# tk1363704/CAREL-VAE

Hardware: AMD Instinct MI355X
Metric: clause-pairs/sec (training step) (higher is better)
Workload: dtype bf16

## Files before the change

carel_vae_amd/csrc/carel_hip_internal.h:

```cpp
#pragma once
#include <hip/hip_runtime.h>
#include <stdarg.h>
#include <stdio.h>
#include "../../include/carel_hip.h"
#include "carel_common.h"

#ifdef CAREL_EXPERIMENTS
#define CAREL_TUNABLE(type, name, value) static type name = value
#else
#define CAREL_TUNABLE(type, name, value) static constexpr type name = value
#endif

namespace carel {

int set_error(int code, const char* fmt, ...);
int check_launch(const char* what);
int slab_reduce_multi(const void* slabs, void* out, int64_t n, const void* slabs2, void* out2, int64_t n2, int splits, const void* partials,
                      int nparts, void* dgamma, void* dbeta, void* dbias, hipStream_t stream);
#ifdef CAREL_EXPERIMENTS
int gemm_rowln_wanted(long rows);
int gemm_rowln_wanted_k(int K);
#else
inline int gemm_rowln_wanted(long) { return 0; }
inline int gemm_rowln_wanted_k(int) { return 0; }
#endif
void encoder_ln_resid_enable(int on);
void encoder_ln_slab_fusion_enable(int on);
void encoder_wgrad_group_enable(int on);
void adam_grid_cap(long cap);
void tail_overlap_enable(int on);
int gemm_pp_init_device(int device);
int gather_rows(const void* in_f32, const void* in_bf16, const void* idx, int n, void* out_f32, void* out_bf16, hipStream_t stream);
int scatter_rows(const void* in_f32, const void* in_bf16, const void* idx, int n, void* out_f32, void* out_bf16, hipStream_t stream);

int layernorm_bwd_rows(const void* dy, const void* h, const void* stats, const void* gamma, int64_t rows, uint32_t drop_seed, uint32_t drop_site,
                       uint32_t drop_idx_offset, float drop_p, const void* drop_row_map, void* dh_f32, void* dy_bf16, void* partials,
                       hipStream_t stream);
int layernorm_bwd_reduce(const void* partials, int64_t rows, void* dgamma, void* dbeta, void* dbias, hipStream_t stream);
int layernorm_bwd_blocks_max(int64_t rows);
int layernorm_bwd_rows_slabs(const void* slabs, int splits, const void* resid, const void* h, const void* stats, const void* gamma, int64_t rows,
                             uint32_t drop_seed, uint32_t drop_site, uint32_t drop_idx_offset, float drop_p, const void* drop_row_map, void* dh_f32,
                             void* dy_bf16, void* partials, hipStream_t stream);
int layernorm_fwd_slabs(const void* slabs, int splits, const void* bias, const void* resid, const void* resid_stats, const void* resid_gamma,
                        const void* resid_beta, uint32_t drop_seed, uint32_t drop_site, uint32_t drop_idx_offset, float drop_p, const void* drop_row_map,
                        void* h_out, const void* gamma, const void* beta, float eps, int64_t rows, void* x_f32, void* x_bf16, void* stats,
                        hipStream_t stream);

constexpr int GEMM_EX_FIXED_ROWS = 0x100;
constexpr int GEMM_EX_DEFER_EPILOGUE = 0x200;
int gemm_bf16_ex(const carel_gemm_args* a, int split_tile_factor, void* stream);
int gemm_bf16_split_plan(const carel_gemm_args* a, int split_tile_factor);
int gemm_wgrad_splits_max(int M, int N, long T);
int embed_ln_bwd_ex(const carel_embed_args* a, const void* dx0, void* dword, void* dpos, void* dtype_, void* dgamma, void* dbeta,
                    void* partials, void* row_scratch, hipStream_t stream, const void* sort_ws = nullptr);
int embed_sort_supported(const carel_embed_args* a);
size_t embed_sort_bytes();
int embed_ln_fwd_keys(const carel_embed_args* a, void* sort_ws, hipStream_t stream);
int embed_sort_rows(const carel_embed_args* a, void* sort_ws, hipStream_t stream);

struct WgradGroupProb { const void* dY; const void* X; void* dW; void* db; int M, N; };
struct WgradGroupLn { const void* partials; int nparts; void* dgamma; void* dbeta; void* dbias; };
size_t gemm_pp_wgrad_group_ws_bytes(const WgradGroupProb* pb, int n, long T);
int gemm_pp_wgrad_group_ok(const WgradGroupProb* pb, int n, long T);
int gemm_pp_wgrad_group(const WgradGroupProb* pb, int n, long T, void* ws, size_t ws_bytes, const WgradGroupLn* ln, int n_ln, hipStream_t stream);

inline Dropout make_dropout(uint32_t seed, uint32_t site, float p, uint32_t idx_offset) {
  Dropout d;
  d.key = mix32(seed + site * 0x9E3779B9u);
  d.idx_offset = idx_offset;
  if (p <= 0.f) { d.thresh = 0u; d.scale = 1.f; }
  else if (p >= 1.f) { d.thresh = 0xFFFFFFFFu; d.scale = 0.f; }
  else {
    d.thresh = (uint32_t)((double)p * 4294967296.0);
    d.scale = (float)(1.0 / (1.0 - (double)p));
    if (d.thresh == 0u) d.scale = 1.f;
  }
  return d;
}

struct AttnParams;
int attn_long_fwd(const AttnParams& q, hipStream_t stream);
int attn_long_bwd(const AttnParams& q, void* workspace, int64_t workspace_bytes, hipStream_t stream);

}
```

carel_vae_amd/csrc/encoder.hip:

```cpp
#include <cstdlib>
#include <mutex>
#include <vector>
#include "carel_hip_internal.h"

using namespace carel;

namespace {

constexpr int EH = 768, EI = 3072, ENH = 12;

size_t al(size_t x) { return (x + 255) & ~(size_t)255; }

struct LayerAct {
  char* xin_bf16; char* qkv; char* lse; char* ctx; char* h1; char* st1; char* x1_bf16; char* u; char* g; char* h2; char* st2;
};
struct ActLayout {
  size_t per_layer, total;
  size_t o_xin, o_qkv, o_lse, o_ctx, o_h1, o_st1, o_x1, o_u, o_g, o_h2, o_st2;
  size_t o_embst, o_xa, o_xb, o_cctx, o_cxres, o_layers;
};

ActLayout act_layout(long B, long S, int L, int inference) {
  const size_t T = (size_t)B * S;
  ActLayout a; size_t o = 0;
// ... 303 lines not shown
    char* next_bf16 = nullptr;
    if (i + 1 < a->n_layers) next_bf16 = layer_act(l, base, i + 1, a->inference).xin_bf16 + (size_t)r0 * EH * 2;
    if (fuse_ln && gemm_rowln_wanted_k(EI)) {
      if ((rc = linear_ln(la.g, w.ffn2_w, EI, w.ffn2_b, xb, 3 + 3 * i, w.ln2_g, w.ln2_b, a->inference ? nullptr : la.h2, xa, next_bf16, la.st2))) return rc;
    } else if ((rc = linear_then_ln(la.g, w.ffn2_w, EI, w.ffn2_b, lnres2 ? (const void*)la.h1 : (const void*)xb, lnres2 ? &lr2 : nullptr, 3 + 3 * i, w.ln2_g,
                                    w.ln2_b, la.h2, need_xa ? xa : nullptr, next_bf16, la.st2))) return rc;
  }
  return CAREL_OK;
}

struct EmbedKeyRecord { const void* scratch; const void* act; const void* ids; const void* tok_row; long rows; bool side; };
static std::mutex g_key_mu;
static std::vector<EmbedKeyRecord> g_key_records;

static long embed_rows_of(const carel_embed_args& e) { return (e.tok_row && e.n_rows > 0) ? (long)e.n_rows : (long)e.batch * e.seq_len; }

static void embed_keys_written(const carel_encoder_args* a, const carel_embed_args* e, bool keys, bool side) {
  std::lock_guard<std::mutex> lk(g_key_mu);
  std::vector<EmbedKeyRecord>& r = g_key_records;
  for (size_t i = 0; i < r.size();)
    if (r[i].act == a->act || (keys && r[i].scratch == a->scratch)) { r[i] = r.back(); r.pop_back(); } else ++i;
  if (keys) r.push_back(EmbedKeyRecord{a->scratch, a->act, a->input_ids, a->tok_row, embed_rows_of(*e), side});
}

static int embed_keys_match(const carel_encoder_args* a, const carel_embed_args* e, bool* side) {
  std::lock_guard<std::mutex> lk(g_key_mu);
  for (const EmbedKeyRecord& k : g_key_records)
    if (k.scratch == a->scratch) {
      *side = k.side;
      return k.act == a->act && k.ids == a->input_ids && k.tok_row == a->tok_row && k.rows == embed_rows_of(*e);
    }
  return 0;
}

extern "C" int carel_encoder_forward(const carel_encoder_args* a, void* stream) {
  int rc = enc_check(a, "carel_encoder_forward");
  if (rc) return rc;
  if (!a->word_emb || !a->pos_emb || !a->type_emb || !a->emb_ln_g || !a->emb_ln_b) return set_error(CAREL_ERR_ARG, "carel_encoder_forward: null embedding tensor");
  const long B = a->batch, S = a->seq_len;
  const ActLayout l = act_layout(B, S, a->n_layers, a->inference);
  const ScratchLayout sl = scratch_layout(B, S);
  char* ws = a->scratch ? (char*)a->scratch + sl.o_ws : nullptr;
  const size_t ws_bytes = a->scratch ? sl.ws_bytes : 0;
  LayerAct la = layer_act(l, (char*)a->act, 0, a->inference);
  carel_embed_args e = embed_args_of(a, l, la);
  if (!a->inference && a->scratch && embed_sort_supported(&e)) {
    void* sort_ws = (char*)a->scratch + sl.o_sort;
    if ((rc = embed_ln_fwd_keys(&e, sort_ws, (hipStream_t)stream))) return rc;
    SideStream* ss = ((a->overlap_wgrad & 1) && !(a->overlap_wgrad & 2)) ? side_stream() : nullptr;
    if (ss) {
      if (hipEventRecord(ss->ev[8], (hipStream_t)stream) != hipSuccess || hipStreamWaitEvent(ss->stream, ss->ev[8], 0) != hipSuccess)
        return set_error(CAREL_ERR_HIP, "carel_encoder_forward: event fork failed");
      if ((rc = embed_sort_rows(&e, sort_ws, ss->stream))) return rc;
    } else if ((rc = embed_sort_rows(&e, sort_ws, (hipStream_t)stream))) return rc;
    embed_keys_written(a, &e, true, ss != nullptr);
  } else {
    embed_keys_written(a, &e, false, false);
    if ((rc = carel_embed_ln_fwd(&e, stream))) return rc;
  }
  const long hb = B / 2;
  const int lsplit = a->n_cls > 0 ? a->n_layers - 1 : a->n_layers;
  SideStream* sd = nullptr;
  if ((a->overlap_wgrad & 2) && !a->tok_row && (B & 1) == 0 && (hb * S) % 128 == 0 && lsplit >= 1 && a->scratch) sd = side_stream();
  if (!sd) return forward_layers(a, 0, a->n_layers, 0, B, stream, ws, ws_bytes);
  if (hipEventRecord(sd->ev[0], (hipStream_t)stream) != hipSuccess || hipStreamWaitEvent(sd->peer, sd->ev[0], 0) != hipSuccess)
    return set_error(CAREL_ERR_HIP, "carel_encoder_forward: event fork failed");
  char* ws2 = (char*)a->scratch + sl.o_slabs;
  rc = forward_layers(a, 0, lsplit, hb, hb, (void*)sd->peer, ws2, sl.ws_bytes, 2);
  if (!rc) rc = forward_layers(a, 0, lsplit, 0, hb, stream, ws, ws_bytes, 2);
  if (rc) return rc;
  if (hipEventRecord(sd->ev[1], sd->peer) != hipSuccess || hipStreamWaitEvent((hipStream_t)stream, sd->ev[1], 0) != hipSuccess)
    return set_error(CAREL_ERR_HIP, "carel_encoder_forward: event join failed");
  if (lsplit < a->n_layers) return forward_layers(a, lsplit, a->n_layers, 0, B, stream, ws, ws_bytes);
  return CAREL_OK;
}

extern "C" int carel_encoder_backward_layer(const carel_encoder_args* a, int32_t layer, void* stream) {
  int rc = enc_check(a, "carel_encoder_backward_layer");
  if (rc) return rc;
  if (a->inference) return set_error(CAREL_ERR_ARG, "carel_encoder_backward_layer: forward ran in inference mode (no saved activations)");
  if (layer < 0 || layer >= a->n_layers || !a->layer_grads || !a->scratch || !a->dx)
    return set_error(CAREL_ERR_ARG, "carel_encoder_backward_layer: bad layer index or null buffer");
  const long B = a->batch, S = a->seq_len, T = n_rows_of(a);
  const ActLayout l = act_layout(B, S, a->n_layers, 0);
  const LayerAct la = layer_act(l, (char*)a->act, layer, 0);
  const ScratchLayout sl = scratch_layout(B, S);
  const int par = layer & 1;
  const Scratch s = scratch_of(sl, (char*)a->scratch, par);
  const carel_layer_params& w = a->layers[layer];
  const carel_layer_grads& g = a->layer_grads[layer];
  const uint32_t hoff = a->drop_row_offset * (uint32_t)(S * EH), aoff = a->drop_row_offset * (uint32_t)(ENH * S * S);
  const size_t ws_bytes = sl.ws_bytes;
  SideStream* sd = nullptr;
  if (a->overlap_wgrad & 1) {
    sd = side_stream();
    if (!sd) return set_error(CAREL_ERR_HIP, "carel_encoder_backward_layer: could not create the side stream / events");
  }
  void* wstream = sd ? (void*)sd->stream : stream;
  int nfork = 0;
  auto fork = [&]() -> int {
    if (!sd) return CAREL_OK;
    hipEvent_t ev = sd->ev[nfork++];
    if (hipEventRecord(ev, (hipStream_t)stream) != hipSuccess || hipStreamWaitEvent(sd->stream, ev, 0) != hipSuccess)
      return set_error(CAREL_ERR_HIP, "carel_encoder_backward_layer: event fork failed");
    return CAREL_OK;
  };
// ... 18 lines not shown
  ga.ln[0] = carel_ln_partial_set{s.part, R, g.ln2_g, g.ln2_b, g.ffn2_b};
  ga.ln[1] = carel_ln_partial_set{s.part3, R, g.ln1_g, g.ln1_b, g.out_b};
  ga.n_ln = 2;
  bool grouped = false;
  if (wgrad_group_enabled() && !cls_only) {
    const int64_t need = carel_gemm_wgrad_group_ws_bytes(&ga);
    grouped = need >= 0 && need <= (int64_t)sl.slab_bytes;
  }
  GemmCall gqkv = gemm_fill(s.dqkv, w.qkv_w, 3 * EH, EH, (int)T, EH, 3 * EH, CAREL_GEMM_NN, CAREL_EPI_ADD_F32, 1, nullptr, nullptr, a->dx, nullptr, s.dy,
                            nullptr, 0, 0, 0, 0.f, nullptr, nullptr, s.ws, ws_bytes, 1);
  const int qkv_slabs = ln_slab_fusion_enabled() ? gemm_bf16_split_plan(&gqkv.g, gqkv.flags) : 1;
  const bool dx_in_slabs = qkv_slabs > 1 && layer + 1 < a->n_layers && !(a->n_cls > 0 && layer + 2 == a->n_layers);
  if ((rc = wait_group(0))) return rc;
  if (dx_in_slabs) {
    if ((rc = layernorm_bwd_rows_slabs(s.ws, qkv_slabs, s.dy, la.h2, la.st2, w.ln2_g, R, a->drop_seed, 3 + 3 * layer, hoff, a->hidden_dropout, rmap, s.dy,
                                       s.dyb, s.part, (hipStream_t)stream))) return rc;
  } else if ((rc = layernorm_bwd_rows(a->dx, la.h2, la.st2, w.ln2_g, R, a->drop_seed, 3 + 3 * layer, hoff, a->hidden_dropout, rmap, s.dy, s.dyb,
                               s.part, (hipStream_t)stream))) return rc;
  if (!grouped) {
    if ((rc = fork())) return rc;
    const LnPartials lp2{s.part, R, g.ln2_g, g.ln2_b, g.ffn2_b};
    if ((rc = wgrad_call(s.dyb, la.g, R, EH, EI, s.slabs, g.ffn2_w, wstream, nullptr, &lp2))) return rc;
    if ((rc = group_done(0))) return rc;
  }
  if ((rc = wait_group(1))) return rc;
  if ((rc = gemm_run(gemm_fill(s.dyb, w.ffn2_w, EH, EI, (int)R, EI, EH, CAREL_GEMM_NN, CAREL_EPI_MUL_BF16, 1, s.du, nullptr, nullptr, nullptr,
                               nullptr, la.u, 0, 0, 0, 0.f, nullptr), stream))) return rc;
  if (!grouped) {
    if ((rc = fork())) return rc;
    if ((rc = wgrad_call(s.du, la.x1_bf16, R, EI, EH, s.slabs, g.ffn1_w, wstream, g.ffn1_b))) return rc;
    if ((rc = group_done(1))) return rc;
  }
  int ffn1_slabs;
  if ((rc = gemm_run_ln(gemm_fill(s.du, w.ffn1_w, EI, EH, (int)R, EH, EI, CAREL_GEMM_NN, CAREL_EPI_ADD_F32, 1, nullptr, nullptr, a->dx, nullptr, s.dy, nullptr,
                                  0, 0, 0, 0.f, nullptr, nullptr, s.ws, ws_bytes, 1 | (cls_only ? GEMM_EX_FIXED_ROWS : 0)),
                        ln_slab_fusion_enabled() && !cls_only, stream, &ffn1_slabs))) return rc;
  if ((rc = wait_group(2))) return rc;
  if (ffn1_slabs > 1) {
    if ((rc = layernorm_bwd_rows_slabs(s.ws, ffn1_slabs, s.dy, la.h1, la.st1, w.ln1_g, R, a->drop_seed, 2 + 3 * layer, hoff, a->hidden_dropout, rmap, s.dy,
                                       s.dyb2, s.part3, (hipStream_t)stream))) return rc;
  } else if ((rc = layernorm_bwd_rows(a->dx, la.h1, la.st1, w.ln1_g, R, a->drop_seed, 2 + 3 * layer, hoff, a->hidden_dropout, rmap, s.dy, s.dyb2,
                               s.part3, (hipStream_t)stream))) return rc;
  void* dctx_rows = cls_only ? (void*)s.dqkv : (void*)s.dctx;
  if (!grouped) {
    if ((rc = fork())) return rc;
    const LnPartials lp1{s.part3, R, g.ln1_g, g.ln1_b, g.out_b};
    if ((rc = wgrad_call(s.dyb2, ctx_rows, R, EH, EH, s.slabs, g.out_w, wstream, nullptr, &lp1))) return rc;
    if ((rc = group_done(2))) return rc;
  }
  if (cls_only && (rc = wait_group(3))) return rc;
  if ((rc = gemm_run(gemm_fill(s.dyb2, w.out_w, EH, EH, (int)R, EH, EH, CAREL_GEMM_NN, CAREL_EPI_BIAS_BF16, 1, dctx_rows, nullptr, nullptr, nullptr,
                               nullptr, nullptr, 0, 0, 0, 0.f, nullptr, nullptr, s.ws, ws_bytes, 1 | (cls_only ? GEMM_EX_FIXED_ROWS : 0)), stream))) return rc;
  if (cls_only) {
    hipError_t he = hipMemsetAsync(s.dctx, 0, (size_t)T * EH * 2, (hipStream_t)stream);
    if (he == hipSuccess) he = hipMemsetAsync(a->dx, 0, (size_t)T * EH * 4, (hipStream_t)stream);
    if (he != hipSuccess) return set_error(CAREL_ERR_HIP, "carel_encoder_backward_layer: memset: %s", hipGetErrorString(he));
    if ((rc = scatter_rows(nullptr, s.dqkv, a->cls_rows, (int)R, nullptr, s.dctx, (hipStream_t)stream))) return rc;
    if ((rc = scatter_rows(s.dy, nullptr, a->cls_rows, (int)R, a->dx, nullptr, (hipStream_t)stream))) return rc;
  }
  const void* dh1_full = cls_only ? (const void*)a->dx : (const void*)s.dy;
  carel_attn_args at;
  at.qkv = la.qkv; at.attention_mask = a->attention_mask; at.ctx = la.ctx; at.lse = la.lse; at.dctx = s.dctx; at.dqkv = s.dqkv;
  at.batch = (int)B; at.seq_len = (int)S; at.heads = ENH; at.head_dim = 64;
  at.drop_seed = a->drop_seed; at.drop_site = 1 + 3 * layer; at.drop_idx_offset = aoff; at.drop_p = a->attn_dropout;
  at.cu_seqlens = a->cu_seqlens;
  at.rel_bias_dist = a->rel_bias_dist; at.d_rel_bias_dist = a->d_rel_bias_dist;
  at.q_rows = cls_only ? 32 : 0;
  at.workspace = (char*)a->scratch + sl.o_attn; at.workspace_bytes = (int64_t)sl.attn_bytes;
  if (a->tok_row && layer + 2 >= a->n_layers) {
    hipError_t he = hipMemsetAsync(s.dqkv + (size_t)(T - 128) * 3 * EH * 2, 0, (size_t)128 * 3 * EH * 2, (hipStream_t)stream);
    if (he != hipSuccess) return set_error(CAREL_ERR_HIP, "carel_encoder_backward_layer: memset: %s", hipGetErrorString(he));
  }
  if ((rc = wait_group(3))) return rc;
  if ((rc = carel_attention_bwd(&at, stream))) return rc;
  if ((rc = fork())) return rc;
  if (grouped) { if ((rc = carel_gemm_wgrad_group(&ga, wstream))) return rc; }
  else if ((rc = wgrad_call(s.dqkv, la.xin_bf16, T, 3 * EH, EH, s.slabs, g.qkv_w, wstream, g.qkv_b))) return rc;
  const bool defer_qkv = qkv_slabs > 1 && layer > 0 && !cls_only;
  gqkv.g.resid_f32 = dh1_full;
  if ((rc = gemm_bf16_ex(&gqkv.g, gqkv.flags | (defer_qkv ? GEMM_EX_DEFER_EPILOGUE : 0), stream))) return rc;
  if (!grouped && (rc = group_done(3))) return rc;
  if (sd) {
    if (hipEventRecord(sd->ev[10 + par], sd->stream) != hipSuccess || hipStreamWaitEvent((hipStream_t)stream, sd->ev[10 + (par ^ 1)], 0) != hipSuccess)
      return set_error(CAREL_ERR_HIP, "carel_encoder_backward_layer: event record / wait failed");
  }
  return CAREL_OK;
}

extern "C" int carel_encoder_backward_join(const carel_encoder_args* a, void* stream) {
  if (!a) return set_error(CAREL_ERR_ARG, "carel_encoder_backward_join: null args");
  if (!(a->overlap_wgrad & 1)) return CAREL_OK;
  SideStream* sd = side_stream();
  if (!sd) return set_error(CAREL_ERR_HIP, "carel_encoder_backward_join: no side stream");
  hipEvent_t ev = sd->ev[SideStream::NEV - 1];
  if (hipEventRecord(ev, sd->stream) != hipSuccess || hipStreamWaitEvent((hipStream_t)stream, ev, 0) != hipSuccess)
    return set_error(CAREL_ERR_HIP, "carel_encoder_backward_join: event join failed");
  return CAREL_OK;
}

extern "C" int carel_encoder_backward_embeddings(const carel_encoder_args* a, void* stream) {
  int rc = enc_check(a, "carel_encoder_backward_embeddings");
  if (rc) return rc;
  if ((rc = carel_encoder_backward_join(a, stream))) return rc;
  if (a->inference || !a->scratch || !a->dx || !a->d_word_emb || !a->d_pos_emb || !a->d_type_emb || !a->d_emb_ln_g || !a->d_emb_ln_b)
    return set_error(CAREL_ERR_ARG, "carel_encoder_backward_embeddings: null buffer or inference-mode forward");
  const long B = a->batch, S = a->seq_len;
  const ActLayout l = act_layout(B, S, a->n_layers, 0);
  const LayerAct la = layer_act(l, (char*)a->act, 0, 0);
  const Scratch s = scratch_of(scratch_layout(B, S), (char*)a->scratch);
  carel_embed_args e = embed_args_of(a, l, la);
  hipError_t he = hipMemsetAsync(a->d_word_emb, 0, (size_t)a->vocab_size * EH * 4, (hipStream_t)stream);
  if (he == hipSuccess) he = hipMemsetAsync(a->d_pos_emb, 0, (size_t)a->max_pos * EH * 4, (hipStream_t)stream);
  if (he != hipSuccess) return set_error(CAREL_ERR_HIP, "carel_encoder_backward_embeddings: memset: %s", hipGetErrorString(he));
  const ScratchLayout sl = scratch_layout(B, S);
  bool side = false;
  const bool keyed = embed_sort_supported(&e) && embed_keys_match(a, &e, &side);
  if (keyed && side && !(a->overlap_wgrad & 1)) {
    SideStream* sd = side_stream();
    if (!sd) return set_error(CAREL_ERR_HIP, "carel_encoder_backward_embeddings: no side stream");
    hipEvent_t ev = sd->ev[SideStream::NEV - 1];
    if (hipEventRecord(ev, sd->stream) != hipSuccess || hipStreamWaitEvent((hipStream_t)stream, ev, 0) != hipSuccess)
      return set_error(CAREL_ERR_HIP, "carel_encoder_backward_embeddings: event join failed");
  }
  const void* sort_ws = keyed ? (const char*)a->scratch + sl.o_sort : nullptr;
  return embed_ln_bwd_ex(&e, a->dx, a->d_word_emb, a->d_pos_emb, a->d_type_emb, a->d_emb_ln_g, a->d_emb_ln_b, s.part, s.dy, (hipStream_t)stream, sort_ws);
}

namespace {

__global__ __launch_bounds__(64) void attn_f32_kernel(const float* __restrict__ qkv, const long* __restrict__ mask, const float* __restrict__ rel,
                                                      float* __restrict__ ctx, int S) {
  const int lane = threadIdx.x;
  const int q = blockIdx.x % S, h = (blockIdx.x / S) % ENH, b = blockIdx.x / (S * ENH);
  __shared__ float qs[64], ps[128];
  const float* base = qkv + (long)b * S * (3 * EH);
  qs[lane] = base[(long)q * (3 * EH) + h * 64 + lane];
  __syncthreads();
  float sc[2], mx = -INFINITY;
#pragma unroll
  for (int i = 0; i < 2; ++i) {
    const int k = lane + i * 64;
    sc[i] = -INFINITY;
    if (k < S && (!mask || mask[(long)b * S + k] != 0)) {
      const float* kr = base + (long)k * (3 * EH) + EH + h * 64;
      float d = 0.f;
      for (int e = 0; e < 64; ++e) d = fmaf(qs[e], kr[e], d);
      d *= 0.125f;
      if (rel) d += rel[h * 256 + 127 + k - q];
      sc[i] = d;
    }
    mx = fmaxf(mx, sc[i]);
  }
#pragma unroll
  for (int o = 32; o > 0; o >>= 1) mx = fmaxf(mx, __shfl_xor(mx, o, 64));
  float pr[2], sum = 0.f;
#pragma unroll
  for (int i = 0; i < 2; ++i) {
    const int k = lane + i * 64;
    pr[i] = k < S ? (mx == -INFINITY ? 1.f : expf(sc[i] - mx)) : 0.f;
    sum += pr[i];
  }
#pragma unroll
  for (int o = 32; o > 0; o >>= 1) sum += __shfl_xor(sum, o, 64);
  ps[lane] = pr[0] / sum; ps[lane + 64] = pr[1] / sum;
  __syncthreads();
  float acc = 0.f;
  for (int k = 0; k < S; ++k) acc = fmaf(ps[k], base[(long)k * (3 * EH) + 2 * EH + h * 64 + lane], acc);
  ctx[((long)b * S + q) * EH + h * 64 + lane] = acc;
}

__global__ __launch_bounds__(256) void gelu_f32_kernel(float* __restrict__ u, long n) {
  const long i = (long)blockIdx.x * 256 + threadIdx.x;
  if (i < n) { const float x = u[i]; u[i] = 0.5f * x * (1.f + erff(x * 0.70710678118654752440f)); }
}

struct F32Work { float *x, *x1, *h, *ctx, *qkv, *u, *stats; char* xb; size_t total; };
F32Work f32_work(char* base, long B, long S) {
  const size_t T = (size_t)B * S;
// ... 54 lines not shown
```

carel_vae_amd/csrc/ln.hip:

```cpp
#include "carel_hip_internal.h"
#include "ln_device.h"
#include "reduce_device.h"

namespace carel {

__global__ __launch_bounds__(256) void ln_fwd_kernel(const float* __restrict__ h, const float* __restrict__ gamma,
                                                     const float* __restrict__ beta, float eps, long rows,
                                                     float* __restrict__ x_f32, bf16_t* __restrict__ x_bf16,
                                                     float* __restrict__ stats) {
  const int lane = threadIdx.x & 63;
  const long row = (long)blockIdx.x * 4 + (threadIdx.x >> 6);
  if (row >= rows) return;
  Row X = load_row(h + row * H, lane);
  const Row G = load_row(gamma, lane), Bt = load_row(beta, lane);
  float mean, rstd;
  ln_normalise(X, G, Bt, eps, mean, rstd);
  if (x_f32) store_row(x_f32 + row * H, lane, X);
  if (x_bf16) store_row_bf16(x_bf16 + row * H, lane, X);
  if (stats && lane == 0) { stats[row * 2] = mean; stats[row * 2 + 1] = rstd; }
}

struct LnFwdSlabs {
  const float* slabs; int splits; long plane;
  const float* bias; const float* resid; const float* resid_stats; const float* resid_gamma; const float* resid_beta;
// ... 394 lines not shown
#pragma unroll
  for (int e = 0; e < 8; ++e) lds[rl][cg * 8 + e] = acc[e];
  __syncthreads();
  const int c = threadIdx.x;
  if (blockIdx.x * 256 + c < n) {
    float s = 0.f;
#pragma unroll
    for (int r = 0; r < 8; ++r) s += lds[r][c];
    partials[(long)blockIdx.y * n + blockIdx.x * 256 + c] = s;
  }
}

__global__ __launch_bounds__(256) void gather_rows_kernel(const float* __restrict__ in_f, const bf16_t* __restrict__ in_b,
                                                          const int* __restrict__ idx, int n, float* __restrict__ out_f,
                                                          bf16_t* __restrict__ out_b) {
  const int lane = threadIdx.x & 63;
  const int i = blockIdx.x * 4 + (threadIdx.x >> 6);
  if (i >= n) return;
  const long r = idx[i];
  if (in_f) {
    Row X;
    if (r >= 0) X = load_row(in_f + r * H, lane);
    else for (int v = 0; v < NV; ++v) X.v[v] = float4{0.f, 0.f, 0.f, 0.f};
    store_row(out_f + (long)i * H, lane, X);
  }
  if (in_b) {
#pragma unroll
    for (int v = 0; v < NV; ++v) {
      const int c = (v * 64 + lane) * 4;
      uint2 x = {0u, 0u};
      if (r >= 0) x = *(const uint2*)(in_b + r * H + c);
      *(uint2*)(out_b + (long)i * H + c) = x;
    }
  }
}
__global__ __launch_bounds__(256) void scatter_rows_kernel(const float* __restrict__ in_f, const bf16_t* __restrict__ in_b,
                                                           const int* __restrict__ idx, int n, float* __restrict__ out_f,
                                                           bf16_t* __restrict__ out_b) {
  const int lane = threadIdx.x & 63;
  const int i = blockIdx.x * 4 + (threadIdx.x >> 6);
  if (i >= n) return;
  const long r = idx[i];
  if (r < 0) return;
  if (in_f) store_row(out_f + r * H, lane, load_row(in_f + (long)i * H, lane));
  if (in_b) {
#pragma unroll
    for (int v = 0; v < NV; ++v) {
      const int c = (v * 64 + lane) * 4;
      *(uint2*)(out_b + r * H + c) = *(const uint2*)(in_b + (long)i * H + c);
    }
  }
}

int gather_rows(const void* in_f32, const void* in_bf16, const void* idx, int n, void* out_f32, void* out_bf16, hipStream_t stream) {
  hipLaunchKernelGGL(gather_rows_kernel, dim3((n + 3) / 4), dim3(256), 0, stream, (const float*)in_f32, (const bf16_t*)in_bf16,
                     (const int*)idx, n, (float*)out_f32, (bf16_t*)out_bf16);
  return check_launch("gather_rows_kernel");
}
int scatter_rows(const void* in_f32, const void* in_bf16, const void* idx, int n, void* out_f32, void* out_bf16, hipStream_t stream) {
  hipLaunchKernelGGL(scatter_rows_kernel, dim3((n + 3) / 4), dim3(256), 0, stream, (const float*)in_f32, (const bf16_t*)in_bf16,
                     (const int*)idx, n, (float*)out_f32, (bf16_t*)out_bf16);
  return check_launch("scatter_rows_kernel");
}

}

using namespace carel;

static EmbedArgs make_embed(const carel_embed_args* a) {
  EmbedArgs e;
  e.ids = (const long*)a->input_ids; e.tt = (const long*)a->token_type_ids;
  e.word = (const float*)a->word_emb; e.pos = (const float*)a->pos_emb; e.type = (const float*)a->type_emb;
  e.gamma = (const float*)a->ln_gamma; e.beta = (const float*)a->ln_beta;
  e.eps = a->ln_eps; e.S = a->seq_len; e.roberta = a->roberta; e.pad_id = a->pad_id;
  e.tok_row = (const int*)a->tok_row;
  e.rows = (a->tok_row && a->n_rows > 0) ? (long)a->n_rows : (long)a->batch * a->seq_len;
  e.vocab = a->vocab_size; e.max_pos = a->max_pos; e.type_vocab = a->type_vocab;
  e.drop = make_dropout(a->drop_seed, 0u, a->drop_p, a->drop_idx_offset);
  return e;
}

static int embed_check(const carel_embed_args* a, const char* who) {
  if (!a) return set_error(CAREL_ERR_ARG, "%s: null args", who);
  if (a->hidden != H) return set_error(CAREL_ERR_SHAPE, "%s: hidden must be %d (got %d)", who, H, a->hidden);
  if (!a->input_ids || !a->word_emb || !a->pos_emb || !a->type_emb || !a->ln_gamma || !a->ln_beta)
    return set_error(CAREL_ERR_ARG, "%s: null tensor", who);
  if (a->batch <= 0 || a->seq_len <= 0 || a->type_vocab < 1 || a->type_vocab > 2)
    return set_error(CAREL_ERR_SHAPE, "%s: bad batch/seq_len/type_vocab", who);
  const long pos_limit = a->roberta ? (long)a->max_pos - a->pad_id - 1 : (long)a->max_pos;
  if (a->seq_len > pos_limit)
    return set_error(CAREL_ERR_SHAPE, "%s: seq_len %d runs past the position table (max_pos %d%s: at most %ld positions)", who, a->seq_len,
                     a->max_pos, a->roberta ? ", ids from pad_id + 1" : "", pos_limit);
  return CAREL_OK;
}

extern "C" int carel_embed_ln_fwd(const carel_embed_args* a, void* stream_) {
  hipStream_t stream = (hipStream_t)stream_;
  int rc = embed_check(a, "carel_embed_ln_fwd");
  if (rc) return rc;
  if (!a->x_f32 || !a->x_bf16 || !a->stats) return set_error(CAREL_ERR_ARG, "carel_embed_ln_fwd: null output");
  EmbedArgs e = make_embed(a);
  hipLaunchKernelGGL(embed_fwd_kernel, dim3((unsigned)((e.rows + 3) / 4)), dim3(256), 0, stream, e, (float*)a->x_f32,
                     (bf16_t*)a->x_bf16, (float*)a->stats, (int2*)nullptr);
  return check_launch("embed_fwd_kernel");
}

// ... 181 lines not shown
```

carel_vae_amd/csrc/tail.hip:

```cpp
#include "carel_hip_internal.h"
#include "mmd_device.h"
#include "hsic_device.h"
#include "rowvec_device.h"
#include "tail_device.h"

namespace carel {

#define TAIL_STAMP(i) do { if (a.prof && threadIdx.x == 0) a.prof[i] = (long long)wall_clock64(); } while (0)

struct MmdGlobalArgs {
  const float* zg; int n, B, D, rank_stride, row_offset;
  float alpha, eps, gscale;
  float* part;
  float* dz;
};
template <int CD>
__global__ __launch_bounds__(256) void mmd_global_kernel(MmdGlobalArgs a) {
  constexpr int CH = 256, ZS = CD + 1;
  __shared__ float zc[CH * ZS];
  __shared__ float nc[CH];
  __shared__ float red[64];
  const int t = threadIdx.x, grp = t & 7;
  const int n = a.n, n2 = 2 * n, D = a.D, D2 = 2 * D;
  auto zrow = [&](int r) -> const float* {
// ... 327 lines not shown
    float m = -INFINITY;
    for (int c = lane; c < chunks; c += 64) m = fmaxf(m, part[((long)c * B + b) * 2]);
    m = wave_max(m);
    float s = 0.f;
    for (int c = lane; c < chunks; c += 64) s += part[((long)c * B + b) * 2 + 1] * expf(part[((long)c * B + b) * 2] - m);
    s = wave_sum(s);
    if (lane == 0) { rowstat[b * 4] = m; rowstat[b * 4 + 1] = logf(s); }
  } else {
    float le = 0.f, dt = 0.f;
    for (int c = lane; c < chunks; c += 64) { le += part[((long)c * B + b) * 2]; dt += part[((long)c * B + b) * 2 + 1]; }
    le = wave_sum(le); dt = wave_sum(dt);
    if (lane == 0) { rowstat[b * 4 + 2] = dt; rowstat[b * 4 + 3] = le; }
  }
}
__global__ __launch_bounds__(256) void decoder_total_kernel(const float* __restrict__ rowstat, int B, float inv_bv, float* __restrict__ terms) {
  __shared__ float red[16];
  float tot = 0.f;
  for (int b = threadIdx.x; b < B; b += 256) tot += rowstat[b * 4 + 3];
  tot = block_sum(tot, red);
  if (threadIdx.x == 0) { terms[7] = tot * inv_bv; terms[8] = terms[0] + tot * inv_bv; }
}

__global__ __launch_bounds__(256) void reduce_parts16_kernel(const float* __restrict__ parts, float* __restrict__ out, int n, int nparts) {
  __shared__ float lds[256];
  const int cl = threadIdx.x & 15, rl = threadIdx.x >> 4;
  const int c = blockIdx.x * 16 + cl;
  float s = 0.f;
  if (c < n) for (int p = rl; p < nparts; p += 16) s += parts[(long)p * n + c];
  lds[threadIdx.x] = s;
  __syncthreads();
  if (rl == 0 && c < n) {
    float t = 0.f;
#pragma unroll
    for (int r = 0; r < 16; ++r) t += lds[r * 16 + cl];
    out[c] = t;
  }
}

__global__ __launch_bounds__(256) void tail_dlat_kernel(const float* __restrict__ dz_core, const float* __restrict__ dz_part, int chunks,
                                                        const float* __restrict__ dlat_direct, const float* __restrict__ lat,
                                                        const float* __restrict__ eps_e, const float* __restrict__ eps_c, int B, int D,
                                                        float gout, float* __restrict__ dlat) {
  const int e = blockIdx.x * 256 + threadIdx.x;
  if (e >= B * 2 * D) return;
  const int b = e / (2 * D), k = e - b * 2 * D;
  float g = dz_core[e];
  for (int c = 0; c < chunks; ++c) g += dz_part[(long)c * B * 2 * D + e];
  const int side = k >= D, kk = k - side * D;
  const float* row = lat + (long)b * 4 * D;
  const float ep = side ? eps_c[kk] : eps_e[kk];
  const float lv = row[(2 * side + 1) * D + kk];
  dlat[(long)b * 4 * D + 2 * side * D + kk] = (dlat_direct[(long)b * 4 * D + 2 * side * D + kk] + g) * gout;
  dlat[(long)b * 4 * D + (2 * side + 1) * D + kk] = (dlat_direct[(long)b * 4 * D + (2 * side + 1) * D + kk] + g * ep * expf(lv)) * gout;
}

__global__ __launch_bounds__(256) void sample_z_kernel(const float* __restrict__ lat, const float* __restrict__ eps_e,
                                                       const float* __restrict__ eps_c, int B, int D, float* __restrict__ z) {
  const int e = blockIdx.x * 256 + threadIdx.x;
  if (e >= B * 2 * D) return;
  const int b = e / (2 * D), k = e - b * 2 * D;
  z[e] = sample_z(lat + (long)b * 4 * D, eps_e, eps_c, D, k);
}

__global__ __launch_bounds__(256) void pair_prob_kernel(const float* __restrict__ lat, const float* __restrict__ eps_e,
                                                        const float* __restrict__ eps_c, const float* __restrict__ w,
                                                        const float* __restrict__ bias, int B, int D, float* __restrict__ prob) {
  const int b = blockIdx.x * 256 + threadIdx.x;
  if (b >= B) return;
  const float* row = lat + (long)b * 4 * D;
  float s = bias[0];
  for (int k = 0; k < D; ++k) {
    s = fmaf(w[k], reparam(row[k], eps_e[k], row[D + k]), s);
    s = fmaf(w[D + k], reparam(row[2 * D + k], eps_c[k], row[3 * D + k]), s);
  }
  prob[b] = 1.0f / (1.0f + expf(-s));
}

constexpr int TT_R = 64;
constexpr int TT_THREADS = 256;
constexpr int TT_MAX_B = 1024;
constexpr int TT_MAX_SLABS = TT_MAX_B / TT_R;
constexpr int TT_MAX_NHW = HeadLayout(8, 32).n;

struct TailTiled {
  TailCore c;
  float* lg;
  float* spart;
  float* hpart;
};

template <int PHASE>
__global__ __launch_bounds__(TT_THREADS) void tail_heads_kernel(TailTiled q) {
  const TailCore& a = q.c;
  extern __shared__ __attribute__((aligned(16))) char smem_raw[];
  float* red = (float*)smem_raw;
  const int B = a.B, D = a.D, D2 = 2 * a.D, D4 = 4 * a.D;
  float* zl = red + 64;
  float* mlt = zl + TT_R * D2;
  float* lg = mlt + TT_R * D4;
  float* elog = lg + TT_R * 16;
  float* gx = elog + TT_R * 8;
  float* hw = gx + TT_R * 2;
  const HeadLayout L(a.EC, D);
  const int t = threadIdx.x;
  const int r0 = blockIdx.x * TT_R, nr = min(TT_R, B - r0);
  const int nslab = gridDim.x;
// ... 392 lines not shown
  const int B = a->batch, D = a->ec_dim, V = a->bow_dim;
  const int nm = (c.z_global && c.dis_mode != 0) ? c.n_global : B;
  const size_t lds = tail_core_lds_bytes(B, D, a->e_classes, nm);
  if (lds > TAIL_LDS_MAX) return set_error(CAREL_ERR_SHAPE, "carel_tail_losses: batch too large for the single-workgroup tail (%zu B LDS)", lds);
  if (lds > 64 * 1024) {
    hipError_t e = hipFuncSetAttribute((const void*)tail_core_kernel, hipFuncAttributeMaxDynamicSharedMemorySize, (int)lds);
    if (e != hipSuccess) return set_error(CAREL_ERR_HIP, "carel_tail_losses: hipFuncSetAttribute: %s", hipGetErrorString(e));
  }
  const int chunks = (V + DEC_J - 1) / DEC_J;
  const DecPlan dp = tail_decoder_plan(B, D);
  if (dp.ldsmax > TAIL_LDS_MAX) return set_error(CAREL_ERR_SHAPE, "carel_tail_losses: batch too large for the decoder kernel (%zu B LDS)", dp.ldsmax);
  if (dp.ldsmax > 64 * 1024) {
    hipError_t e = hipSuccess;
    for (auto& family : DEC_WG)
      for (auto kernel : family)
        if (e == hipSuccess) e = hipFuncSetAttribute((const void*)kernel, hipFuncAttributeMaxDynamicSharedMemorySize, (int)dp.ldsmax);
    if (e != hipSuccess) return set_error(CAREL_ERR_HIP, "carel_tail_losses: hipFuncSetAttribute: %s", hipGetErrorString(e));
  }
  c.mmd_part = nullptr; c.mmd_nblk = 0; c.dz_mmd = nullptr;
  if (c.z_global && c.dis_mode == 0 && (2 * c.n_global + 31) / 32 > MMD_MAX_BLOCKS)
    return set_error(CAREL_ERR_SHAPE, "carel_tail_losses: global batch too large for the MMD partial buffer");
  hipStream_t core_stream = stream;
  TailEvents* tev = nullptr;
  auto join_on_error = [&](int code) -> int {
    if (tev && core_stream != stream) {
      (void)hipEventRecord(tev->join, core_stream);
      (void)hipStreamWaitEvent(stream, tev->join, 0);
    }
    return code;
  };
  if (g_tail_overlap && !a->serial && !g_tail_prof) {
    hipStream_t side = (hipStream_t)carel_side_stream(0);
    tev = side ? tail_events() : nullptr;
    if (tev) {
      hipLaunchKernelGGL(sample_z_kernel, dim3((B * 2 * D + 255) / 256), dim3(256), 0, stream, c.lat, c.eps_e, c.eps_c, B, D, c.z);
      if (hipEventRecord(tev->fork, stream) != hipSuccess || hipStreamWaitEvent(side, tev->fork, 0) != hipSuccess)
        return set_error(CAREL_ERR_HIP, "carel_tail_losses: event fork failed");
      core_stream = side;
      c.z = nullptr;
    }
  }
  if (c.z_global && c.dis_mode == 0) {
    if ((rc = launch_mmd_global(c, w, c.z_global, c.n_global, c.rank_stride, c.row_offset, core_stream))) return join_on_error(rc);
  }
  c.prof = g_tail_prof;
  hipLaunchKernelGGL(tail_core_kernel, dim3(1), dim3(1024), lds, core_stream, c);
  if ((rc = check_launch("tail_core_kernel"))) return join_on_error(rc);
  if (tev && hipEventRecord(tev->join, core_stream) != hipSuccess) return join_on_error(set_error(CAREL_ERR_HIP, "carel_tail_losses: event record failed"));

  const DecArgs d = dec_args(a, w);
  const size_t dec_lds[3] = {dp.lds1, dp.lds2, dp.lds3};
  launch_decoder(DEC_WG, d, dim3(chunks), dim3(chunks), DEC_J * dp.G, dec_lds, stream);
  if ((rc = check_launch("decoder kernels"))) return join_on_error(rc);
  launch_dz_reduce(a, w, stream);
  if (tev && hipStreamWaitEvent(stream, tev->join, 0) != hipSuccess) return join_on_error(set_error(CAREL_ERR_HIP, "carel_tail_losses: event join failed"));
  return launch_tail_close(a, w, d.gscale, stream);
}

extern "C" int carel_tail_losses_tiled(const carel_tail_args* a, void* stream_) {
  hipStream_t stream = (hipStream_t)stream_;
  const char* who = "carel_tail_losses_tiled";
  if (!a) return set_error(CAREL_ERR_ARG, "%s: null args", who);
  if (a->batch > TT_MAX_B) return set_error(CAREL_ERR_SHAPE, "%s: batch must be <= %d; got %d", who, TT_MAX_B, a->batch);
  TailTiled q; TailWork w;
  TailCore& c = q.c;
  int rc = tail_losses_prepare(a, who, c, w);
  if (rc) return rc;
  const int B = a->batch, D = a->ec_dim, V = a->bow_dim;
  if (c.dis_mode == 1)
    return set_error(CAREL_ERR_SHAPE, "%s: HSIC (dis_mode 1) keeps the single-workgroup limit of carel_tail_losses: batch <= %d at ec_dim %d, "
                     "e_classes %d; got %d", who, (int)carel_tail_batch_limit(D, a->e_classes), D, a->e_classes, B);
  const int nm = c.z_global ? c.n_global : B;
  const int nblk = (2 * nm + 31) / 32;
  if (c.dis_mode == 0 && nblk > MMD_MAX_BLOCKS) return set_error(CAREL_ERR_SHAPE, "%s: global batch too large for the MMD partial buffer", who);
  const int nslab = (B + TT_R - 1) / TT_R;
  const int n_hw = HeadLayout(a->e_classes, D).n;
  const size_t lds_h = sizeof(float) * (64 + (size_t)TT_R * (2 * D + 4 * D + 16 + 8 + 2) + ((n_hw + 3) & ~3));
  const int D2 = 2 * D, chunks = (V + DEC_J - 1) / DEC_J;
  auto dec_lds = [&](int tb, int tiles) { return sizeof(float) * ((size_t)tb * D2 + ((DEC_J * (D2 + 1) + 3) & ~3) + (size_t)tiles * tb * DEC_J); };
  const int TB = dec_lds(32, 2) <= 64 * 1024 ? 32 : 16;
  if (lds_h > 64 * 1024 || dec_lds(TB, 2) > 64 * 1024 || nslab > TT_MAX_SLABS || n_hw > TT_MAX_NHW)
    return set_error(CAREL_ERR_SHAPE, "%s: internal tile plan does not fit (ec_dim %d, e_classes %d)", who, D, a->e_classes);
  const int ntile = (B + TB - 1) / TB;
  q.lg = w.tt_lg; q.spart = w.tt_spart; q.hpart = w.tt_hpart;

  hipLaunchKernelGGL(sample_z_kernel, dim3((B * 2 * D + 255) / 256), dim3(256), 0, stream, c.lat, c.eps_e, c.eps_c, B, D, c.z);
  if (c.dis_mode == 0) {
    rc = c.z_global ? launch_mmd_global(c, w, c.z_global, nm, c.rank_stride, c.row_offset, stream)
                    : launch_mmd_global(c, w, c.z, nm, B * 2 * D, 0, stream);
    if (rc) return rc;
  }
  hipLaunchKernelGGL(tail_heads_kernel<1>, dim3(nslab), dim3(TT_THREADS), lds_h, stream, q);
  hipLaunchKernelGGL(tail_heads_kernel<2>, dim3(nslab), dim3(TT_THREADS), lds_h, stream, q);
  hipLaunchKernelGGL(tail_head_grads_kernel, dim3(1), dim3(TT_THREADS), 0, stream, q, nslab);
  if ((rc = check_launch("tail_heads_kernel"))) return rc;

  const DecArgs d = dec_args(a, w);
  const size_t lds_d[3] = {dec_lds(TB, 1), dec_lds(TB, 2), dec_lds(TB, 1)};
  launch_decoder(DEC_TILED, d, dim3(chunks, ntile), dim3(chunks), DEC_J * DEC_MAXG, lds_d, stream, TB);
  if ((rc = check_launch("decoder kernels (tiled)"))) return rc;
  launch_dz_reduce(a, w, stream);
  return launch_tail_close(a, w, d.gscale, stream);
}

extern "C" int carel_scale_f32(void* x, int64_t n, const void* scale_dev, void* stream_) {
  hipStream_t stream = (hipStream_t)stream_;
  if (!x || !scale_dev || n <= 0) return set_error(CAREL_ERR_ARG, "carel_scale_f32: bad arguments");
  long blocks = (n + 255) / 256; if (blocks > 2048) blocks = 2048;
  hipLaunchKernelGGL(scale_inplace_kernel, dim3((unsigned)blocks), dim3(256), 0, stream, (float*)x, (long)n, (const float*)scale_dev);
// ... 106 lines not shown
```

carel_vae_amd/drl_classifier.py:

```python
import ctypes as C
import math
import os
from types import SimpleNamespace

import numpy as np
import torch
import torch.nn as nn

from . import _lib as L
from . import ops

H, I_FF, NH = 768, 3072, 12

DEFAULT_OPT = dict(language="zh", max_len=128, e_num_class=6, c_num_class=1, pair_num_class=1, ec_dim=24, bert_dim=768,
                   kl_ann_iterations=20000, epochs=20, batch_size=64, ec_kl_lambda=0.03, label_smoothing=0.1,
                   mmd_loss_weight=30.0, emo_mul_loss_weight=10.0, cau_mul_loss_weight=10.0, pair_mul_loss_weight=30.0,
                   dropout=0.5, epsilon=1e-8, vae_lr=1e-5, aprx_lr=0.003, pair_bow_dim=23771, self_iteration=50, self_epochs=10,
                   self_strategy="random", best_model_path="ECPE_model/best_cause_pair_model", model_id="carel")


def make_opt(**kw):
    d = dict(DEFAULT_OPT)
    d.update(kw)
    return SimpleNamespace(**d)
# ... 992 lines not shown
        prev = self._flat_grad.clone() if accumulate else None
        if accumulate and self._gan:
            prev[self._disc_lo:self._disc_hi].zero_()
        go = grad_out.to(torch.float32).reshape(1).contiguous()
        ea = c.ea
        ea.dx = c.buf.dx_last.data_ptr()
        ops.tail_backward(c.ta, go, None if grad_z is None else grad_z.to(torch.float32).contiguous())
        if c.ad is not None:
            c.ad.dx_f32 = ea.dx
            ops.adapter_backward(c.ad)
            if self._adapter_train_names:
                ops.adapter_backward_weights(c.ad, ops.adapter_wgrad_args(self._ws[("adapter", c.B, c.S)], self._adapter_grads()))
        lo = self._offs["decoder.weight"]
        ops.scale_(self._flat_grad[lo:self._pair_hi], go)
        if self._dp is not None:
            self._dp.tail_done()
        self._backward_encoder(ea, accumulate)
        if c.ad is not None:
            e = "encoder.embeddings."
            self._grad_view(e + "word_embeddings.weight")[self.cfg.pad_id].zero_()
            if self.cfg.roberta:
                self._grad_view(e + "position_embeddings.weight")[self.cfg.pad_id].zero_()
        if self._dp is not None:
            self._dp.backward_done(None if accumulate else self._adam_hook)
        if accumulate:
            self._flat_grad.add_(prev)
        self._bind_grads()
        if self.strict_pair_skip and self._has_pair_skip and not accumulate:
            off = L.load().carel_tail_pair_dead_offset(c.B, self.opt.ec_dim, self.opt.pair_bow_dim)
            if float(c.buf.work[off]) != 0.0:
                for k in self._pair_range_names:
                    self._named[k].grad = None

    def _backward_encoder(self, ea, accumulate):
        lib = L.load()
        st = L.current_stream()

        def layer_ready(l):
            work = self._dp.layer_done(l) if self._dp is not None else None
            if self._adam_hook is not None and not accumulate and (self._dp is None or work is not None):
                self._adam_hook._layer_ready(l, after=work)

        span = rel_span(int(ea.seq_len))
        rel = self._rel_buffers(int(ea.batch), span) if getattr(self.cfg, "rel_pos", False) else None
        if rel is not None:
            if rel.ddist.data_ptr() != ea.d_rel_bias_dist:
                raise L.CarelError("internal: the relative-position gradient buffer was re-allocated between forward and backward")
            rel.ddist[:int(ea.batch) * NH].zero_()
        lag = 1 if self.overlap_wgrad else 0
        for l in range(self.cfg.layers - 1, -1, -1):
            L.check(lib.carel_encoder_backward_layer(C.byref(ea), l, st), "carel_encoder_backward_layer")
            if l + lag < self.cfg.layers:
                layer_ready(l + lag)
        if lag:
            L.check(lib.carel_encoder_backward_join(C.byref(ea), st), "carel_encoder_backward_join")
            layer_ready(0)
        L.check(lib.carel_encoder_backward_embeddings(C.byref(ea), st), "carel_encoder_backward_embeddings")
        if rel is not None:
            L.check(lib.carel_relpos_reduce_span(rel.ddist.data_ptr(), int(ea.batch), rel.bucket.data_ptr(), self._g(REL_KEY), 0, span, st),
                    "carel_relpos_reduce_span")

    def _bind_grads(self):
        if self._grad_views is None:
            self._grad_views = {k: self._grad_view(k) for k in self._order}
        skip = set(self._aprx_names) | (set(self._adapter_names) - set(self._adapter_train_names)) | set(self._disc_names)
        for k, p in self._named.items():
            if k not in skip:
                p.grad = self._grad_views[k]

    def forward(self, input_ids, att_masks, token_type_ids, emotion_labels, cause_labels, pair_labels, content_bow, iteration,
                seq_lengths=None):
        c = self._make_call(input_ids, att_masks, token_type_ids, emotion_labels, cause_labels, pair_labels, content_bow, iteration,
                            training=torch.is_grad_enabled(), seq_lengths=seq_lengths)
        self._last_call = c
        vi = bool(self._aprx_names)
        D = self.opt.ec_dim
        if self._gan:
            if torch.is_grad_enabled():
                return _GanLosses.apply(self._flat.new_zeros((), requires_grad=True), self, c)
            self._run_forward(c, training=False)
            t = c.gan_terms
            return t[0].clone(), t[1].clone(), t[4].clone()
        if torch.is_grad_enabled():
            anchor = self._flat.new_zeros((), requires_grad=True)
            loss, z = _TrainLoss.apply(anchor, self, c)
            c.z_out = z
            if vi:
                z_e, z_c = z[:, :D], z[:, D:]
                return z_e, z_c, self.get_ec_aprx_loss(z_e, z_c), loss
            return loss
        self._run_forward(c, training=False)
        loss = c.buf.terms[8].clone()
        if vi:
            z = c.buf.z.clone()
            return z[:, :D], z[:, D:], self.get_ec_aprx_loss(z[:, :D], z[:, D:]), loss
        return loss

    def sampled_embeddings(self):
        z = self._last_call.z_out
        D = self.opt.ec_dim
        return z[:, :D], z[:, D:]

    def forward_terms(self, *args, **kw):
        with torch.no_grad():
            self.forward(*args, **kw)
        c = self._last_call
        t = c.buf.terms.clone()
        D = self.opt.ec_dim
        lat = c.buf.lat.clone()
        out = {n: t[i] for i, n in enumerate(self.TERM_NAMES)}
# ... 196 lines not shown
```

Measured before the change: 8467.

## Fuse CLS-only backward scatter, reorder embedding backward before join, fuse tail close

In the CLS-only last-layer backward, two full memsets plus scatters are replaced by a tile kernel that writes only the needed rows of dctx. dx is now fed by adding the CLS rows after the QKV gemm, with the gemm residual set to null. Embedding backward now runs before the wgrad side-stream join, using an event recorded after the embedding sort, so it can overlap with deferred weight-gradient work. In the tail, the dz reduction and tail-close kernels are merged into one kernel. Several ordering and correctness assumptions change: dx must already be initialised before add_rows, and the tile kernel only covers the first 32 rows of each sequence.

```diff
diff --git a/carel_vae_amd/csrc/carel_hip_internal.h b/carel_vae_amd/csrc/carel_hip_internal.h
--- a/carel_vae_amd/csrc/carel_hip_internal.h
+++ b/carel_vae_amd/csrc/carel_hip_internal.h
@@ -32,6 +32,8 @@
 int gemm_pp_init_device(int device);
 int gather_rows(const void* in_f32, const void* in_bf16, const void* idx, int n, void* out_f32, void* out_bf16, hipStream_t stream);
 int scatter_rows(const void* in_f32, const void* in_bf16, const void* idx, int n, void* out_f32, void* out_bf16, hipStream_t stream);
+int add_rows(const void* in_f32, const void* idx, int n, void* out_f32, hipStream_t stream);
+int cls_tile_rows(const void* in_bf16, const void* idx, const void* cu_seqlens, int batch, int seq_len, long rows, void* out_bf16, hipStream_t stream);
 
 int layernorm_bwd_rows(const void* dy, const void* h, const void* stats, const void* gamma, int64_t rows, uint32_t drop_seed, uint32_t drop_site,
                        uint32_t drop_idx_offset, float drop_p, const void* drop_row_map, void* dh_f32, void* dy_bf16, void* partials,
diff --git a/carel_vae_amd/csrc/encoder.hip b/carel_vae_amd/csrc/encoder.hip
--- a/carel_vae_amd/csrc/encoder.hip
+++ b/carel_vae_amd/csrc/encoder.hip
@@ -379,6 +379,7 @@
       if (hipEventRecord(ss->ev[8], (hipStream_t)stream) != hipSuccess || hipStreamWaitEvent(ss->stream, ss->ev[8], 0) != hipSuccess)
         return set_error(CAREL_ERR_HIP, "carel_encoder_forward: event fork failed");
       if ((rc = embed_sort_rows(&e, sort_ws, ss->stream))) return rc;
+      if (hipEventRecord(ss->ev[9], ss->stream) != hipSuccess) return set_error(CAREL_ERR_HIP, "carel_encoder_forward: event record failed");
     } else if ((rc = embed_sort_rows(&e, sort_ws, (hipStream_t)stream))) return rc;
     embed_keys_written(a, &e, true, ss != nullptr);
   } else {
@@ -503,13 +504,15 @@
   if ((rc = gemm_run(gemm_fill(s.dyb2, w.out_w, EH, EH, (int)R, EH, EH, CAREL_GEMM_NN, CAREL_EPI_BIAS_BF16, 1, dctx_rows, nullptr, nullptr, nullptr,
                                nullptr, nullptr, 0, 0, 0, 0.f, nullptr, nullptr, s.ws, ws_bytes, 1 | (cls_only ? GEMM_EX_FIXED_ROWS : 0)), stream))) return rc;
   if (cls_only) {
-    hipError_t he = hipMemsetAsync(s.dctx, 0, (size_t)T * EH * 2, (hipStream_t)stream);
-    if (he == hipSuccess) he = hipMemsetAsync(a->dx, 0, (size_t)T * EH * 4, (hipStream_t)stream);
-    if (he != hipSuccess) return set_error(CAREL_ERR_HIP, "carel_encoder_backward_layer: memset: %s", hipGetErrorString(he));
-    if ((rc = scatter_rows(nullptr, s.dqkv, a->cls_rows, (int)R, nullptr, s.dctx, (hipStream_t)stream))) return rc;
-    if ((rc = scatter_rows(s.dy, nullptr, a->cls_rows, (int)R, a->dx, nullptr, (hipStream_t)stream))) return rc;
-  }
-  const void* dh1_full = cls_only ? (const void*)a->dx : (const void*)s.dy;
+    if (S <= 128) {
+      if ((rc = cls_tile_rows(s.dqkv, a->cls_rows, a->cu_seqlens, (int)B, (int)S, T, s.dctx, (hipStream_t)stream))) return rc;
+    } else {
+      hipError_t he = hipMemsetAsync(s.dctx, 0, (size_t)T * EH * 2, (hipStream_t)stream);
+      if (he != hipSuccess) return set_error(CAREL_ERR_HIP, "carel_encoder_backward_layer: memset: %s", hipGetErrorString(he));
+      if ((rc = scatter_rows(nullptr, s.dqkv, a->cls_rows, (int)R, nullptr, s.dctx, (hipStream_t)stream))) return rc;
+    }
+  }
+  const void* dh1_full = cls_only ? nullptr : (const void*)s.dy;
   carel_attn_args at;
   at.qkv = la.qkv; at.attention_mask = a->attention_mask; at.ctx = la.ctx; at.lse = la.lse; at.dctx = s.dctx; at.dqkv = s.dqkv;
   at.batch = (int)B; at.seq_len = (int)S; at.heads = ENH; at.head_dim = 64;
@@ -530,6 +533,7 @@
   const bool defer_qkv = qkv_slabs > 1 && layer > 0 && !cls_only;
   gqkv.g.resid_f32 = dh1_full;
   if ((rc = gemm_bf16_ex(&gqkv.g, gqkv.flags | (defer_qkv ? GEMM_EX_DEFER_EPILOGUE : 0), stream))) return rc;
+  if (cls_only && (rc = add_rows(s.dy, a->cls_rows, (int)R, a->dx, (hipStream_t)stream))) return rc;
   if (!grouped && (rc = group_done(3))) return rc;
   if (sd) {
     if (hipEventRecord(sd->ev[10 + par], sd->stream) != hipSuccess || hipStreamWaitEvent((hipStream_t)stream, sd->ev[10 + (par ^ 1)], 0) != hipSuccess)
@@ -552,29 +556,29 @@
 extern "C" int carel_encoder_backward_embeddings(const carel_encoder_args* a, void* stream) {
   int rc = enc_check(a, "carel_encoder_backward_embeddings");
   if (rc) return rc;
-  if ((rc = carel_encoder_backward_join(a, stream))) return rc;
   if (a->inference || !a->scratch || !a->dx || !a->d_word_emb || !a->d_pos_emb || !a->d_type_emb || !a->d_emb_ln_g || !a->d_emb_ln_b)
     return set_error(CAREL_ERR_ARG, "carel_encoder_backward_embeddings: null buffer or inference-mode forward");
   const long B = a->batch, S = a->seq_len;
   const ActLayout l = act_layout(B, S, a->n_layers, 0);
   const LayerAct la = layer_act(l, (char*)a->act, 0, 0);
-  const Scratch s = scratch_of(scratch_layout(B, S), (char*)a->scratch);
+  const ScratchLayout sl = scratch_layout(B, S);
+  const Scratch s = scratch_of(sl, (char*)a->scratch, 1);
   carel_embed_args e = embed_args_of(a, l, la);
+  bool side = false;
+  const bool keyed = embed_sort_supported(&e) && embed_keys_match(a, &e, &side);
+  if (keyed && side) {
+    SideStream* sd = side_stream();
+    if (!sd) return set_error(CAREL_ERR_HIP, "carel_encoder_backward_embeddings: no side stream");
+    if (hipStreamWaitEvent((hipStream_t)stream, sd->ev[9], 0) != hipSuccess)
+      return set_error(CAREL_ERR_HIP, "carel_encoder_backward_embeddings: event wait failed");
+  }
   hipError_t he = hipMemsetAsync(a->d_word_emb, 0, (size_t)a->vocab_size * EH * 4, (hipStream_t)stream);
   if (he == hipSuccess) he = hipMemsetAsync(a->d_pos_emb, 0, (size_t)a->max_pos * EH * 4, (hipStream_t)stream);
   if (he != hipSuccess) return set_error(CAREL_ERR_HIP, "carel_encoder_backward_embeddings: memset: %s", hipGetErrorString(he));
-  const ScratchLayout sl = scratch_layout(B, S);
-  bool side = false;
-  const bool keyed = embed_sort_supported(&e) && embed_keys_match(a, &e, &side);
-  if (keyed && side && !(a->overlap_wgrad & 1)) {
-    SideStream* sd = side_stream();
-    if (!sd) return set_error(CAREL_ERR_HIP, "carel_encoder_backward_embeddings: no side stream");
-    hipEvent_t ev = sd->ev[SideStream::NEV - 1];
-    if (hipEventRecord(ev, sd->stream) != hipSuccess || hipStreamWaitEvent((hipStream_t)stream, ev, 0) != hipSuccess)
-      return set_error(CAREL_ERR_HIP, "carel_encoder_backward_embeddings: event join failed");
-  }
   const void* sort_ws = keyed ? (const char*)a->scratch + sl.o_sort : nullptr;
-  return embed_ln_bwd_ex(&e, a->dx, a->d_word_emb, a->d_pos_emb, a->d_type_emb, a->d_emb_ln_g, a->d_emb_ln_b, s.part, s.dy, (hipStream_t)stream, sort_ws);
+  if ((rc = embed_ln_bwd_ex(&e, a->dx, a->d_word_emb, a->d_pos_emb, a->d_type_emb, a->d_emb_ln_g, a->d_emb_ln_b, s.part, s.dy, (hipStream_t)stream, sort_ws)))
+    return rc;
+  return carel_encoder_backward_join(a, stream);
 }
 
 namespace {
diff --git a/carel_vae_amd/csrc/ln.hip b/carel_vae_amd/csrc/ln.hip
--- a/carel_vae_amd/csrc/ln.hip
+++ b/carel_vae_amd/csrc/ln.hip
@@ -470,6 +470,48 @@
   }
 }
 
+__global__ __launch_bounds__(256) void add_rows_kernel(const float* __restrict__ in_f, const int* __restrict__ idx, int n, float* __restrict__ out_f) {
+  const int lane = threadIdx.x & 63;
+  const int i = blockIdx.x * 4 + (threadIdx.x >> 6);
+  if (i >= n) return;
+  const long r = idx[i];
+  if (r < 0) return;
+  Row X = load_row(out_f + r * H, lane);
+  const Row D = load_row(in_f + (long)i * H, lane);
+#pragma unroll
+  for (int v = 0; v < NV; ++v) { X.v[v].x += D.v[v].x; X.v[v].y += D.v[v].y; X.v[v].z += D.v[v].z; X.v[v].w += D.v[v].w; }
+  store_row(out_f + r * H, lane, X);
+}
+__global__ __launch_bounds__(256) void cls_tile_rows_kernel(const bf16_t* __restrict__ in_b, const int* __restrict__ idx, const int* __restrict__ cu,
+                                                            int B, int S, long T, bf16_t* __restrict__ out_b) {
+  const int lane = threadIdx.x & 63, wave = threadIdx.x >> 6;
+  const int b = blockIdx.x;
+  const long row0 = cu ? (long)cu[b] : (long)b * S;
+  const long end = cu ? (long)cu[b + 1] : row0 + S;
+  const long used = cu ? (long)cu[B] : T;
+  const long src = idx[b];
+  for (int j = wave; j < 32; j += 4) {
+    const long r = row0 + j;
+    if (r >= T || (r >= end && r < used)) continue;
+#pragma unroll
+    for (int v = 0; v < NV; ++v) {
+      const int c = (v * 64 + lane) * 4;
+      uint2 x = {0u, 0u};
+      if (r == src) x = *(const uint2*)(in_b + (long)b * H + c);
+      *(uint2*)(out_b + r * H + c) = x;
+    }
+  }
+}
+
+int add_rows(const void* in_f32, const void* idx, int n, void* out_f32, hipStream_t stream) {
+  hipLaunchKernelGGL(add_rows_kernel, dim3((n + 3) / 4), dim3(256), 0, stream, (const float*)in_f32, (const int*)idx, n, (float*)out_f32);
+  return check_launch("add_rows_kernel");
+}
+int cls_tile_rows(const void* in_bf16, const void* idx, const void* cu_seqlens, int batch, int seq_len, long rows, void* out_bf16, hipStream_t stream) {
+  hipLaunchKernelGGL(cls_tile_rows_kernel, dim3(batch), dim3(256), 0, stream, (const bf16_t*)in_bf16, (const int*)idx, (const int*)cu_seqlens, batch,
+                     seq_len, rows, (bf16_t*)out_bf16);
+  return check_launch("cls_tile_rows_kernel");
+}
 int gather_rows(const void* in_f32, const void* in_bf16, const void* idx, int n, void* out_f32, void* out_bf16, hipStream_t stream) {
   hipLaunchKernelGGL(gather_rows_kernel, dim3((n + 3) / 4), dim3(256), 0, stream, (const float*)in_f32, (const bf16_t*)in_bf16,
                      (const int*)idx, n, (float*)out_f32, (bf16_t*)out_bf16);
diff --git a/carel_vae_amd/csrc/tail.hip b/carel_vae_amd/csrc/tail.hip
--- a/carel_vae_amd/csrc/tail.hip
+++ b/carel_vae_amd/csrc/tail.hip
@@ -403,6 +403,42 @@
   const float lv = row[(2 * side + 1) * D + kk];
   dlat[(long)b * 4 * D + 2 * side * D + kk] = (dlat_direct[(long)b * 4 * D + 2 * side * D + kk] + g) * gout;
   dlat[(long)b * 4 * D + (2 * side + 1) * D + kk] = (dlat_direct[(long)b * 4 * D + (2 * side + 1) * D + kk] + g * ep * expf(lv)) * gout;
+}
+
+__global__ __launch_bounds__(256) void tail_close_kernel(float* __restrict__ dz_part, int nparts, const float* __restrict__ dz_core,
+                                                         const float* __restrict__ dlat_direct, const float* __restrict__ lat,
+                                                         const float* __restrict__ eps_e, const float* __restrict__ eps_c, int B, int D,
+                                                         const float* __restrict__ rowstat, float inv_bv, float* __restrict__ terms,
+                                                         float* __restrict__ dlat) {
+  __shared__ float lds[256];
+  __shared__ float red[16];
+  const int n = B * 2 * D;
+  const int cl = threadIdx.x & 15, rl = threadIdx.x >> 4;
+  const int c = blockIdx.x * 16 + cl;
+  float s = 0.f;
+  if (c < n) for (int p = rl; p < nparts; p += 16) s += dz_part[(long)p * n + c];
+  lds[threadIdx.x] = s;
+  __syncthreads();
+  if (rl == 0 && c < n) {
+    float t = 0.f;
+#pragma unroll
+    for (int r = 0; r < 16; ++r) t += lds[r * 16 + cl];
+    dz_part[c] = t;
+    const int b = c / (2 * D), k = c - b * 2 * D;
+    const float g = dz_core[c] + t;
+    const int side = k >= D, kk = k - side * D;
+    const float* row = lat + (long)b * 4 * D;
+    const float ep = side ? eps_c[kk] : eps_e[kk];
+    const float lv = row[(2 * side + 1) * D + kk];
+    dlat[(long)b * 4 * D + 2 * side * D + kk] = dlat_direct[(long)b * 4 * D + 2 * side * D + kk] + g;
+    dlat[(long)b * 4 * D + (2 * side + 1) * D + kk] = dlat_direct[(long)b * 4 * D + (2 * side + 1) * D + kk] + g * ep * expf(lv);
+  }
+  if (blockIdx.x == 0) {
+    float tot = 0.f;
+    for (int b = threadIdx.x; b < B; b += 256) tot += rowstat[b * 4 + 3];
+    tot = block_sum(tot, red);
+    if (threadIdx.x == 0) { terms[7] = tot * inv_bv; terms[8] = terms[0] + tot * inv_bv; }
+  }
 }
 
 __global__ __launch_bounds__(256) void sample_z_kernel(const float* __restrict__ lat, const float* __restrict__ eps_e,
@@ -901,9 +937,12 @@
   const size_t dec_lds[3] = {dp.lds1, dp.lds2, dp.lds3};
   launch_decoder(DEC_WG, d, dim3(chunks), dim3(chunks), DEC_J * dp.G, dec_lds, stream);
   if ((rc = check_launch("decoder kernels"))) return join_on_error(rc);
-  launch_dz_reduce(a, w, stream);
   if (tev && hipStreamWaitEvent(stream, tev->join, 0) != hipSuccess) return join_on_error(set_error(CAREL_ERR_HIP, "carel_tail_losses: event join failed"));
-  return launch_tail_close(a, w, d.gscale, stream);
+  const int n = B * 2 * D;
+  hipLaunchKernelGGL(tail_close_kernel, dim3((n + 15) / 16), dim3(256), 0, stream, w.dz_part, chunks, (const float*)w.dz_core,
+                     (const float*)w.dlat_direct, (const float*)a->lat, (const float*)a->eps_e, (const float*)a->eps_c, B, D, (const float*)w.rowstat,
+                     d.gscale, (float*)a->terms, w.dlat);
+  return check_launch("tail_close_kernel");
 }
 
 extern "C" int carel_tail_losses_tiled(const carel_tail_args* a, void* stream_) {
diff --git a/carel_vae_amd/drl_classifier.py b/carel_vae_amd/drl_classifier.py
--- a/carel_vae_amd/drl_classifier.py
+++ b/carel_vae_amd/drl_classifier.py
@@ -1068,10 +1068,9 @@
             L.check(lib.carel_encoder_backward_layer(C.byref(ea), l, st), "carel_encoder_backward_layer")
             if l + lag < self.cfg.layers:
                 layer_ready(l + lag)
+        L.check(lib.carel_encoder_backward_embeddings(C.byref(ea), st), "carel_encoder_backward_embeddings")
         if lag:
-            L.check(lib.carel_encoder_backward_join(C.byref(ea), st), "carel_encoder_backward_join")
             layer_ready(0)
-        L.check(lib.carel_encoder_backward_embeddings(C.byref(ea), st), "carel_encoder_backward_embeddings")
         if rel is not None:
             L.check(lib.carel_relpos_reduce_span(rel.ddist.data_ptr(), int(ea.batch), rel.bucket.data_ptr(), self._g(REL_KEY), 0, span, st),
                     "carel_relpos_reduce_span")
```

New measurement: 8543, median of 6. Within noise of the previous version (+0.9%).
